# Intsights/PySubstringSearch

Hardware: AMD Instinct MI355X
Metric: queries/sec (batched) + index-build GB/s on 512MB chunk, 1/2/4/8 GPU (higher is better)
Workload: dtype u64

## Files before the change

pysubstringsearch_amd/csrc/common.cpp:

```cpp
#include "common.h"
#include "knobs.h"

#include <atomic>
#include <cstring>
#include <cstdio>
#include <cstdlib>
#include <algorithm>
#include <cerrno>
#include <unistd.h>

#include <mutex>
#include <vector>

namespace pss {

static thread_local std::string g_err;

void set_error(const char *fmt, ...)
{
    char buf[1024];
    va_list ap;
    va_start(ap, fmt);
    vsnprintf(buf, sizeof buf, fmt, ap);
    va_end(ap);
// ... 294 lines not shown
    if (e != hipSuccess || count <= 0) {
        (void)hipGetLastError();
        set_error("no usable HIP device (%s); libpss has no CPU fallback",
                  e != hipSuccess ? hipGetErrorString(e) : "device count is 0");
        return PSS_EDEVICE;
    }
    if (device < 0 || device >= count || device >= kMaxDevices) {
        set_error("device %d out of range (have %d)", device, count);
        return PSS_EINVAL;
    }
    PSS_HIP(hipSetDevice(device));
    std::lock_guard<std::mutex> lk(g_ctx_mu);
    DeviceCtx &c = table[device];
    if (c.device < 0) PSS_TRY(init_ctx(c, device));
    *out = &c;
    return PSS_OK;
}

int get_helper_ctx(DeviceCtx *parent, DeviceCtx **out)
{
    if (!parent->helper) {
        DeviceCtx *h = new DeviceCtx();
        const int rc = init_ctx(*h, parent->device);
        if (rc != PSS_OK) {
            delete h;
            return rc;
        }
        parent->helper = h;
    }
    *out = parent->helper;
    return PSS_OK;
}

int get_ctx(int device, DeviceCtx **out) { return get_ctx_of(g_ctx, device, out); }
int get_build_ctx(int device, DeviceCtx **out) { return get_ctx_of(g_bctx, device, out); }

int DeviceCtx::ensure_resident()
{
    if (resident.arena) return PSS_OK;
    PSS_HIP(hipStreamCreateWithFlags(&resident.stream, hipStreamNonBlocking));
    PSS_HIP(hipHostMalloc(&resident.arena, kPinnedBytes, hipHostMallocCoherent | hipHostMallocMapped));
    PSS_HIP(hipHostGetDevicePointer(&resident.arena_dev, resident.arena, 0));
    memset(resident.arena, 0, kPinnedBytes);
    return PSS_OK;
}

void DeviceCtx::Resident::post(const uint8_t *q, uint32_t plen)
{
    ResidentMailbox *mb = reinterpret_cast<ResidentMailbox *>(static_cast<uint8_t *>(arena) + kResidentMailboxOff);
    if (plen != kResidentStop) {
        if (plen <= sizeof mb->post.bytes) {
            memcpy(mb->post.bytes, q, plen);
        } else {
            memcpy(mb->query, q, plen);
            memset(mb->query + plen, 0, 32);
        }
    }
    mb->post.plen = plen;
    ++seq;
    __atomic_store_n(&mb->post.seq_b, seq, __ATOMIC_RELEASE);
    __atomic_store_n(&mb->post.seq_a, seq, __ATOMIC_RELEASE);
}

void DeviceCtx::stop_resident()
{
    if (!resident.running) return;
    resident.post(nullptr, kResidentStop);
    (void)hipStreamSynchronize(resident.stream);
    resident.running = false;
}

const KnobDef kKnobs[] = {
    {"PSS_KEY_CHARS", "0 (chosen)", "1|2|3|5|8|12|16", "builder: force the symbols packed into the initial sort key"},
    {"PSS_KEY_DROP", "-1 (chosen)", "0|1|3|7", "builder: force the low bits of the last key symbol that are left out"},
    {"PSS_NO_SAMPLE", "unset", "1", "builder: size the initial key from symbol counts even for large texts (no sizing sample)"},
    {"PSS_NO_TIES_PASS", "unset", "1", "builder: plain 8-byte-key LSD passes and key comparison in the rerank (no tie flags)"},
    {"PSS_MODE", "chosen", "dense|sparse|text", "builder: how ties are resolved -- doubling over an inverse suffix array, sparse (hash), text rounds"},
    {"PSS_TEXT_ROUNDS", "5", "0|1|2|3", "builder: text rounds at most before the rank rounds"},
    {"PSS_MSD", "-1 (screened)", "0|1|1", "initial sort: never / whenever the key fits the hybrid MSD radix sort (msd_sort.hip)"},
    {"PSS_MSD_LSD", "1", "0|1", "MSD sort: 0 = digits in MSD order with a second histogram pass (rounds 2-5); else LSD order, second pass by look-back"},
    {"PSS_MSD_KEY_CAP", "48", "", "MSD sort: largest key width tried (bits; the element format bounds it further)"},
    {"PSS_MSD_PARTIAL_SYMBOL", "unset", "1", "MSD sort: fill the element with the high bits of one more symbol than fits whole (fewer ties; measured slower on lines)"},
    {"PSS_MSD_NO_FUSE", "unset", "1", "MSD sort: ties flagged in the suffix array instead of emitted from the local sort"},
    {"PSS_MSD_SLOW_LOCAL", "unset", "1", "MSD sort: the general (ballot LSD) local-sort kernel for every tile"},
    {"PSS_MSD_SCATTER", "unset", "1", "MSD sort in MSD order: the 8192-element partition kernels of round 2"},
    {"PSS_SS", "-1 (n >= 2^24, MSD declined)", "0|1", "initial sort: never / whenever the text has the size for it the sample sort over 16-byte elements"},
    {"PSS_SS_SEG", "1", "0", "sample sort: 0 = every tile merge-sorted as one array instead of bucket by bucket"},
    {"PSS_SS_WINDOW_PLAN", "unset", "1", "sample sort: tiles by the window rule of the MSD sort instead of the greedy plan"},
    {"PSS_SS_DEBUG", "unset", "", "sample sort: print where a bucket beyond a tile came from (diagnostic)"},
    {"PSS_NO_PLAN_CACHE", "unset", "1", "builder: forget between chunks which initial sort and alphabet the previous chunk took"},
    {"PSS_NO_PLAN_FRONT", "unset", "1", "builder: remember the sort but not the alphabet (separate alphabet and recode passes)"},
    {"PSS_RLE", "-1 (runs average >= 8 bytes)", "0|1|1", "builder: never / always the run-length path (rle_build.hip)"},
    {"PSS_RLE_SORT", "unset", "1", "run-length path: expansion by the stable radix sort instead of the matrix walk"},
    {"PSS_PERIOD", "-1 (when the text repeats one word)", "0", "builder: 0 = never the closed form for a text that repeats one word"},
    {"PSS_ANCHOR", "-1 (texts of >= 2^20 bytes)", "0|1|1", "builder: never / whenever ties outlive the text rounds the anchor round (anchor_impl.h)"},
    {"PSS_ANCHOR_OMEGA", "0 (as wide as the common prefix allows)", "9|12|17|33", "anchor round: force the window of the minimizers"},
    {"PSS_ANCHOR_MIN_OMEGA", "11", "3|7|9", "anchor round: narrowest window it accepts by itself"},
    {"PSS_ANCHOR_SIDE", "-1 (>= 2^24 bytes, sampled ties show copies)", "0|1", "anchor round: never / always sort the anchors beside the text round (second stream)"},
    {"PSS_ANCHOR_SIDE_PCT", "8", "", "anchor round: share of sampled tied pairs that must be copies for the side line"},
    {"PSS_ANCHOR_CAP_DIV", "5", "3|4", "anchor round: declines above n / this many anchors"},
    {"PSS_NO_PROBE", "unset", "1", "builder: always a text round before the anchor round (no sampling of the ties)"},
    {"PSS_PROBE_SKIP_PCT", "50", "0|20|90", "builder: no text rounds when more than this share of the sampled tied pairs are repeats"},
    {"PSS_NO_MID_TIER", "unset", "1", "rounds: groups above 512 members all take the chained radix sorts"},
    {"PSS_NO_MID_MERGE", "unset", "1", "rounds: groups of 513 .. 4096 members with a crowded bin take the chained sorts (no LDS merge sort)"},
    {"PSS_BIG_MERGE", "-1 (by the average size of the large groups)", "0|1|2", "rounds: groups above 4096 members through the segmented merge sort (2: in text rounds only)"},
    {"PSS_NO_BIG_MERGE", "unset", "", "rounds: overrides PSS_BIG_MERGE"},
    {"PSS_COUNT_SORT", "unset", "1", "rank rounds: groups ranked by counting instead of the merge sort"},
    {"PSS_PERIODIC", "1", "0", "rank rounds: 0 = no periodic keys for the large groups"},
    {"PSS_TIMING", "unset", "", "builder / Writer: per-round and per-stage trace on stderr"},
    {"PSS_DEVICES", "all visible", "0|0,0|0,0,0|all", "devices of Reader(path) / Writer(path) without a device argument: all | comma-separated ordinals"},
    {"PSS_DEVICE", "unset", "", "default device of a process (launchers' LOCAL_RANK etc. are honoured the same way)"},
    {"PSS_IO_THREADS", "8 .. 16 by core count", "2|5", "file path: threads of the I/O pool"},
    {"PSS_INGEST_BLOCK", "32 MiB", "16|40|300", "Writer: size of the direct reads of add_entries_from_file_lines"},
    {"PSS_INGEST_MIN_ROOM", "1 MiB", "1|20", "Writer: room a chunk must have left for one direct read"},
    {"PSS_WRITER_MMAP", "tmpfs: 1, else 0", "0|1", "Writer: records through a shared mapping (1) or pwrite (0)"},
    {"PSS_WRITER_MMAP_MIN", "1 MiB", "16", "Writer: smallest record that goes through the mapping"},
    {"PSS_WRITER_HOST_BUDGET", "8 GiB", "", "multi-device Writer: host text of the chunks in flight (one chunk always goes through)"},
    {"PSS_STRIPES", "8", "", "striped container format 2: stripe files of a Writer"},
    {"PSS_EXPERIMENT_NO_FILE", "unset", "", "measurement only: the record thread copies without writing the file"},
    {"PSS_RESULT_ORDER", "text", "sa", "Reader: 'sa' = the reference's order inside a chunk (suffix-array order of every entry's first hit)"},
    {"PSS_READER_HBM_BUDGET", "whatever hipMalloc grants minus 2 GiB", "", "Reader: suffix arrays beyond this many bytes of HBM stay in pinned host memory"},
    {"PSS_READER_AUTO_RESIDENCY", "1", "", "Reader: 0 = the residency manager never moves a suffix array by itself"},
    {"PSS_NO_KEY_SAMPLES", "unset", "", "Reader: no key-sample table"},
    {"PSS_SAMPLE_SHIFT", "11", "", "Reader: one key sample per 2^shift suffixes"},
    {"PSS_LINE_BLOCK_SHIFT", "8", "6|7|9|10", "Reader: the line index behind entry ids keeps one newline rank per 2^shift bytes of text (6 .. 10)"},
    {"PSS_NO_SMALL_PATH", "unset", "1", "search: no fused single-query kernels"},
    {"PSS_NO_BLOCK_PATH", "unset", "1", "search: small batches one wave per pair instead of one workgroup"},
    {"PSS_NO_SEARCH_STAGE", "unset", "1", "search: no pinned staging of queries and results"},
    {"PSS_WAVE_SEARCH", "unset", "1", "search: interval kernel one wave per pair at every batch size"},
    {"PSS_NO_GROUP_SEARCH", "unset", "1", "search: never 16 lanes per pair"},
    {"PSS_NO_MID_PIPELINE", "unset", "1", "search: always the general multi-kernel pipeline"},
    {"PSS_PINNED_POOL_BYTES", "40 GiB", "", "search: pinned host memory the result pool keeps between batches"},
    {"PSS_NO_PINNED_RESULTS", "unset", "1", "search: large results into pageable memory"},
    {"PSS_LANE_SEARCH_MIN", "8192", "1|100000", "search: pairs from which one lane per pair searches"},
    {"PSS_SEARCH_EVENTS", "unset", "", "single-query path: HIP events around the fused kernel (fills ms_device; ~4 us per query)"},
    {"PSS_RESIDENT_IDLE_US", "1000", "", "low-latency mode: the resident kernel leaves after this long without a query"},
    {"PSS_RESIDENT_LIFE_US", "50000", "", "low-latency mode: ... and after this long in any case"},
    {"PSS_TRACE_RESIDENT", "unset", "", "libpss_trace.so only: print the resident kernel's phase stamps"},
    {"PSS_RCCL_LIB", "librccl.so of the process", "", "gather inside the C ABI: the RCCL library to load"},
    {"PSS_RCCL_TIMEOUT_MS", "60000", "", "gather inside the C ABI: bound of every wait for the peers"},
};
const int kNumKnobs = (int)(sizeof(kKnobs) / sizeof(kKnobs[0]));

const char *knob(const char *name)
{
    for (int i = 0; i < kNumKnobs; ++i)
        if (strcmp(kKnobs[i].name, name) == 0) return getenv(name);
    static std::atomic<bool> said{false};
    if (!said.exchange(true)) fprintf(stderr, "[pss] %s is not in the switch registry (knobs.h): treated as unset\n", name);
    return nullptr;
}

uint64_t workspace_bytes(int device)
{
    if (device < 0 || device >= kMaxDevices) return 0;
    std::lock_guard<std::mutex> lk(g_ctx_mu);
    uint64_t total = 0;
    for (DeviceCtx *table : {g_ctx, g_bctx}) {
        DeviceCtx &c = table[device];
        if (c.device < 0) continue;
        for (auto &s : c.slot) total += s.cap;
        if (c.helper)
            for (auto &s : c.helper->slot) total += s.cap;
    }
    return total;
}
// ... 27 lines not shown
```

pysubstringsearch_amd/csrc/msd_sort.hip:

```cpp
#include "msd_sort.h"

#include <algorithm>
#include <vector>

#include "prims.h"
#include "scan.h"
#include "text_keys.h"

namespace pss {

constexpr int MSD_D = 10;
constexpr u32 MSD_BINS = 1u << MSD_D;
constexpr int MSD_BLOCK = 512;
constexpr int MSD_WAVES = MSD_BLOCK / kWave;
constexpr int MSD_IPT = 16;
constexpr u32 MSD_TILE = MSD_BLOCK * MSD_IPT;
constexpr u32 MSD_WIN = 6144;
#ifndef PSS_LS_WINDOW
#define PSS_LS_WINDOW 8
#endif
constexpr u32 MSD_TILE_CAP = 8184 - PSS_LS_WINDOW;
constexpr u32 MSD_MAX_BUCKET = 4088;
constexpr int MSD_TAG_BITS = MSD_D + 1;
constexpr u32 MSD_TAG_SPAN = 1u << MSD_TAG_BITS;
// ... 522 lines not shown
                        e = ((e >> 24) << a.idx_bits) | (u64)(base + ((u32)e & (MSD_TILE2 - 1u)));
                    } else {
                        d = (u32)(e >> shift2) & (MSD_BINS - 1u);
                        e = (e & low_mask2) | ((u64)(hist[d] >> 16) << shift2);
                    }
                    a.out[s_delta[d] + p] = e;
                }
            }
        }
    }
}

constexpr u32 LB_A = 1u << 30, LB_P = 2u << 30, LB_STATE = 3u << 30, LB_VALUE = LB_A - 1u;
constexpr int LB_WINDOW = 4;

struct LbAsk {
    u32 v[LB_WINDOW];
};
__device__ __forceinline__ void lb_ask(const u32 *status, u32 p, LbAsk &q)
{
#pragma unroll
    for (u32 w = 0; w < (u32)LB_WINDOW; ++w) {
        const u32 r = p > w ? p - 1 - w : 0u;
        q.v[w] = __hip_atomic_load(&status[(size_t)r * MSD_BINS + threadIdx.x], __ATOMIC_RELAXED, __HIP_MEMORY_SCOPE_AGENT);
    }
}
__device__ __forceinline__ void lb_begin(u32 *status, u32 t, u32 c, LbAsk &q)
{
    if (t == 0) return;
    __hip_atomic_store(&status[(size_t)t * MSD_BINS + threadIdx.x], LB_A | c, __ATOMIC_RELAXED, __HIP_MEMORY_SCOPE_AGENT);
    lb_ask(status, t, q);
}
__device__ __forceinline__ u32 lb_finish(u32 *status, u32 t, u32 c, u32 first, LbAsk &q)
{
    u32 off = first;
    if (t != 0) {
        u32 sum = 0, p = t;
        for (;;) {
            const u32 p0 = p;
            bool stop = false, done = false;
#pragma unroll
            for (u32 w = 0; w < (u32)LB_WINDOW; ++w) {
                if (!stop && w < p0) {
                    const u32 st = q.v[w] & LB_STATE;
                    if (st == 0) {
                        stop = true;
                    } else {
                        sum += q.v[w] & LB_VALUE;
                        --p;
                        if (st == LB_P) done = stop = true;
                    }
                }
            }
            if (done || p == 0) break;
            lb_ask(status, p, q);
        }
        off = sum;
    }
    __hip_atomic_store(&status[(size_t)t * MSD_BINS + threadIdx.x], LB_P | (off + c), __ATOMIC_RELAXED, __HIP_MEMORY_SCOPE_AGENT);
    return off;
}


__global__ __launch_bounds__(MSD_BINS) void msd_tiles2_kernel(const u32 *J1, MsdTile2 *tiles, u32 *counters)
{
    __shared__ u32 scr[MSD_BINS / kWave + 1];
    const u32 d = threadIdx.x;
    const u32 s = J1[d], e = J1[d + 1];
    const u32 nr = (e - s + MSD_TILE2 - 1) / MSD_TILE2;
    u32 total = 0, D = 0;
    const u32 first = block_excl_sum<MSD_BINS / kWave>(nr, scr, &total);
    const u32 dn = block_excl_sum<MSD_BINS / kWave>(nr ? 1u : 0u, scr, &D);
    if (d == 0) counters[0] = total + (MSD_BINS - D);
    if (nr == 0) {
        const u32 dd = D + (d - dn);
        tiles[total + (d - dn)] = MsdTile2{s, 0u, dd | 0x80000000u};
    }
    for (u32 k = 0; k < nr; ++k) {
        const u32 ts = s + k * MSD_TILE2;
        tiles[first + k] = MsdTile2{ts, min(MSD_TILE2, e - ts), dn | (k + 1 == nr ? 0x80000000u : 0u)};
    }
}

__global__ __launch_bounds__(1024) void msd_scatter_lb_kernel(MsdArgs a)
{
    constexpr int BLOCK = 1024;
    constexpr int IPT = MSD_TILE2 / BLOCK;
    __shared__ __attribute__((aligned(16))) u64 exch[MSD_TILE];
    __shared__ u32 hist[MSD_BINS], s_delta[MSD_BINS];
    __shared__ u16 s_start[MSD_BINS];
    __shared__ u32 scr[BLOCK / kWave + 1];
    __shared__ u32 s_ticket;
    const u32 tid = threadIdx.x;
    const u32 nt = a.counters[0];
    const int shift2 = a.idx_bits + a.key_bits - 2 * MSD_D;
    const u64 low_mask2 = (1ull << shift2) - 1ull;
    hist[tid] = 0;
    __syncthreads();
    for (;;) {
        if (tid == 0) s_ticket = atomicAdd(&a.counters[8], 1u);
        __syncthreads();
        const u32 t = s_ticket;
        if (t >= nt) break;
        const MsdTile2 td = a.tiles2[t];
        const u32 base = td.start, valid = td.count;
        u64 elem[IPT];
        u32 lp[IPT];
#pragma unroll
        for (int k = 0; k < IPT; ++k) {
            const u32 p = k * BLOCK + tid;
            elem[k] = p < valid ? a.in[base + p] : 0ull;
        }
#pragma unroll
        for (int k = 0; k < IPT; ++k) {
            const u32 p = k * BLOCK + tid;
            const u32 d = (u32)(elem[k] >> shift2) & (MSD_BINS - 1u);
            lp[k] = p < valid ? (atomicAdd(&hist[d], 1u) | (d << 22)) : 0xffffffffu;
        }
        __syncthreads();
        const u32 c = hist[tid];
        LbAsk ask;
        lb_begin(a.status, t, c, ask);
        const u32 ex = block_excl_sum<BLOCK / kWave>(c, scr, nullptr);
        s_start[tid] = (u16)ex;
        hist[tid] = 0;
        __syncthreads();
        const u64 tag = (u64)(td.d_last & (MSD_RAW_TAG_SPAN - 1u)) << shift2;
#pragma unroll
        for (int k = 0; k < IPT; ++k)
            if (lp[k] != 0xffffffffu) lp[k] = (lp[k] & 0xffffu) + (u32)s_start[lp[k] >> 22];
#pragma unroll
        for (int h = 0; h < MSD_PIECES2; ++h) {
            if (h && h * MSD_TILE >= valid) break;
            if (h) __syncthreads();
#pragma unroll
            for (int k = 0; k < IPT; ++k) {
                const u32 q = lp[k] - h * MSD_TILE;
                if (q < MSD_TILE) exch[q] = elem[k];
            }
            if (h == 0) {
                if (t == 0 && tid == 0) a.J[0] = 0;
                const u32 off = lb_finish(a.status, t, c, a.Jb[tid], ask);
                if (td.d_last >> 31) a.J[(size_t)tid * MSD_BINS + (td.d_last & (MSD_BINS - 1u)) + 1u] = off + c;
                s_delta[tid] = off - ex;
            }
            __syncthreads();
#pragma unroll
            for (int k = 0; k < (int)(MSD_TILE / BLOCK); ++k) {
                const u32 q = k * BLOCK + tid, p = h * MSD_TILE + q;
                if (p < valid) {
                    const u64 e = exch[q];
                    const u32 d = (u32)(e >> shift2) & (MSD_BINS - 1u);
                    a.out[s_delta[d] + p] = (e & low_mask2) | tag;
                }
            }
        }
    }
}


struct InNonEmpty {
    const u32 *J;
    __device__ u64 operator()(u64 j) const { return J[j + 1] > J[j] ? 1u : 0u; }
};

__global__ __launch_bounds__(256) void msd_compact_kernel(const u32 *J, u32 nb, const u64 *rank, u32 *cstart, u32 *counters, u32 *cj)
{
    u32 mx = 0;
    for (u32 j = blockIdx.x * blockDim.x + threadIdx.x; j < nb; j += gridDim.x * blockDim.x) {
        const u32 s = J[j], e = J[j + 1];
        if (e > s) {
            cstart[rank[j]] = s;
            if (cj) cj[rank[j]] = j;
            mx = max(mx, e - s);
        }
    }
    mx = wave_incl_max(mx);
    if (lane_id() == kWave - 1 && mx) atomicMax(&counters[1], mx);
}

struct TilePlan {
    u32 win, cap;
    const u32 *cj;
};
__device__ __forceinline__ bool msd_tile_head(const u32 *cstart, u32 ne, u32 n, u32 k, TilePlan tp)
{
    if (tp.cj) {
        if (k == 0 || (tp.cj[k] >> MSD_RAW_TAG_BITS) != (tp.cj[k - 1] >> MSD_RAW_TAG_BITS)) return true;
    } else if ((k & (MSD_TAG_SPAN - 1u)) == 0) {
        return true;
    }
    const u32 w = cstart[k] / tp.win;
    if (cstart[k - 1] / tp.win != w) return true;
    if (k + 1 < ne && cstart[k + 1] / tp.win == w) return false;
    u32 lo = 0, hi = k;
    const u32 ws = w * tp.win;
    while (lo < hi) {
        const u32 mid = (lo + hi) >> 1;
        if (cstart[mid] < ws) lo = mid + 1; else hi = mid;
    }
    const u32 end = k + 1 < ne ? cstart[k + 1] : n;
    return end - cstart[lo] > tp.cap;
}

struct InTileHead {
    const u32 *cstart;
    u32 ne, n;
    TilePlan tp;
    __device__ u64 operator()(u64 k) const { return msd_tile_head(cstart, ne, n, (u32)k, tp) ? 1u : 0u; }
};

struct InTileHeadDev {
    const u32 *cstart;
    const u64 *nep;
    u32 n;
    TilePlan tp;
    __device__ u64 operator()(u64 k) const
    {
        const u32 ne = (u32)*nep;
        return (k < ne && msd_tile_head(cstart, ne, n, (u32)k, tp)) ? 1u : 0u;
    }
};
__global__ __launch_bounds__(256) void msd_tiles_dev_kernel(const u32 *cstart, const u64 *nep, u32 n, const u64 *rank, const u64 *total,
                                                              u32 *tile_first, TilePlan tp)
{
    const u32 ne = (u32)*nep;
    if (blockIdx.x == 0 && threadIdx.x == 0) tile_first[*total] = ne;
    for (u32 k = blockIdx.x * blockDim.x + threadIdx.x; k < ne; k += gridDim.x * blockDim.x) {
        if (msd_tile_head(cstart, ne, n, k, tp)) tile_first[rank[k]] = k;
    }
}

// ... 148 lines not shown
                for (int w = 0; w < MSD_WAVES; ++w) {
                    c[w] = wave_hist[w][tid];
                    total += c[w];
                }
            }
            const u32 incl = wave_incl_sum(total);
            if (lane == kWave - 1) scr[wave] = incl;
            __syncthreads();
            if (tid < 256) {
                u32 run = incl - total;
                for (u32 w = 0; w < wave; ++w) run += scr[w];
#pragma unroll
                for (int w = 0; w < MSD_WAVES; ++w) {
                    wave_hist[w][tid] = run;
                    run += c[w];
                }
            }
        }
        __syncthreads();
#pragma unroll
        for (int r = 0; r < MSD_IPT; ++r) {
            const bool pad = wave * (kWave * MSD_IPT) + r * kWave + lane >= count;
            const u32 d = pad ? dmask : ((u32)(key[r] >> shift) & dmask);
            exch[wave_hist[wave][d] + rank[r]] = key[r];
        }
        __syncthreads();
        for (u32 i = tid; i < MSD_WAVES * 256; i += MSD_BLOCK) (&wave_hist[0][0])[i] = 0;
#pragma unroll
        for (int r = 0; r < MSD_IPT; ++r) key[r] = exch[wave * (kWave * MSD_IPT) + r * kWave + lane];
        __syncthreads();
    }
    if (sort_bits <= 0) {
#pragma unroll
        for (int r = 0; r < MSD_IPT; ++r) exch[wave * (kWave * MSD_IPT) + r * kWave + lane] = key[r];
        __syncthreads();
    }
    if (tid == 0) scr[0] = 0;
    __syncthreads();
    msd_emit_tile(exch, count, e0, idx_bits, sa_out, em, &scr[0]);
    __syncthreads();
    if (em && tid == 0) em->blk_cnt[t] = scr[0];
}


#ifndef PSS_LS_BIN_BITS
#define PSS_LS_BIN_BITS 12
#endif
constexpr int LS_BIN_BITS = PSS_LS_BIN_BITS;
constexpr u32 LS_BINS = 1u << LS_BIN_BITS;
constexpr u32 LS_WORDS = LS_BINS / 2;
constexpr u32 LS_KMAX = 64;
#ifndef PSS_LS_GROUP
#define PSS_LS_GROUP 1
#endif
constexpr int LS_GROUP = PSS_LS_GROUP;
constexpr int LS_WINDOW = PSS_LS_WINDOW;

__global__ __launch_bounds__(256) void msd_tile_desc_kernel(const u32 *cstart, const u32 *tile_first, u32 nt, u32 ne, u32 n,
                                                              MsdTile *tiles, const u32 *cj, const u64 *ntp, const u64 *nep)
{
    const u32 t = blockIdx.x * blockDim.x + threadIdx.x;
    if (ntp) {
        nt = (u32)*ntp;
        ne = (u32)*nep;
    }
    if (t >= nt) return;
    const u32 k0 = tile_first[t], k1 = tile_first[t + 1];
    const u32 e0 = cstart[k0], e1 = k1 < ne ? cstart[k1] : n;
    if (cj) {
        const u32 t0 = cj[k0] & (MSD_RAW_TAG_SPAN - 1u), t1 = cj[k1 - 1] & (MSD_RAW_TAG_SPAN - 1u);
        tiles[t] = MsdTile{e0, e1 - e0, t0, t1 - t0 + 1u};
    } else {
        tiles[t] = MsdTile{e0, e1 - e0, k0 & (MSD_TAG_SPAN - 1u), k1 - k0};
    }
}

__device__ __forceinline__ void keep_load(u64 &v) { asm volatile("" : "+v"(v)); }

__device__ __forceinline__ void lds_barrier()
{
    asm volatile("s_waitcnt lgkmcnt(0)\n\ts_barrier" ::: "memory");
}

__global__ __launch_bounds__(MSD_BLOCK, 4) void msd_local_fast_kernel(const u64 *in, const MsdTile *tiles, u32 nt, int rem_bits,
                                                                     int idx_bits, u32 *sa_out, u32 *fail_list, u32 *fail_count,
                                                                     int fused, MsdEmit em_val, const u64 *nt_dev,
                                                                     const u32 *counters_dev, const u32 *bad_dev)
{
    if (nt_dev) {
        if (counters_dev[1] > MSD_MAX_BUCKET || (bad_dev && *bad_dev)) return;
        nt = (u32)*nt_dev;
    }
    const MsdEmit *em = fused ? &em_val : nullptr;
    __shared__ __attribute__((aligned(16))) u64 lds_all[MSD_TILE + LS_WORDS];
    u64 *const exch = lds_all;
    u32 *const hist = reinterpret_cast<u32 *>(lds_all + MSD_TILE);
    u32 *const hist2 = hist + LS_WORDS;
    u32 *const scr = reinterpret_cast<u32 *>(&exch[MSD_TILE - 8]);
    u32 &s_fail = scr[MSD_WAVES + 2];
    const u32 tid = threadIdx.x;
    const u32 stride = gridDim.x;
    u32 t = blockIdx.x;
    if (t >= nt) return;
    MsdTile cur = tiles[t];
    MsdTile nxt = t + stride < nt ? tiles[t + stride] : MsdTile{0, 0, 0, 0};
    u64 pe[MSD_IPT];
    auto prefetch = [&](const MsdTile &d) {
#pragma unroll
        for (int r = 0; r < MSD_IPT; ++r) {
            const u32 p = r * MSD_BLOCK + tid;
            pe[r] = p < d.count ? in[d.e0 + p] : 0ull;
        }
    };
    prefetch(cur);
    for (u32 i = tid; i < LS_WORDS; i += MSD_BLOCK) hist[i] = 0;
    if (tid == 0) {
        s_fail = 0;
        scr[MSD_WAVES + 3] = 0;
    }
    lds_barrier();
    u32 prev_t = 0;
    bool prev_ok = false;
    for (;;) {
        const u32 count = cur.count, e0 = cur.e0;
        const u32 rows = (count + MSD_BLOCK - 1) / MSD_BLOCK;
        int seg_bits = 0;
        while ((1u << seg_bits) < cur.nb) ++seg_bits;
        const u64 tag_base = (u64)cur.tag0 << (rem_bits + idx_bits);
        const int sort_bits = rem_bits + seg_bits;
        const int bin_shift = idx_bits + (sort_bits > LS_BIN_BITS ? sort_bits - LS_BIN_BITS : 0);
        u64 e[MSD_IPT];
#pragma unroll
        for (int r = 0; r < MSD_IPT; ++r) {
            e[r] = ~0ull;
            if ((u32)r < rows) {
                const u32 p = r * MSD_BLOCK + tid;
                if (p < count) {
                    e[r] = pe[r] - tag_base;
                    const u32 bin = (u32)(e[r] >> bin_shift);
                    atomicAdd(&hist[bin >> 1], 1u << (16u * (bin & 1u)));
                }
            }
        }
        const bool more = t + stride < nt;
        if (more) prefetch(nxt);
        lds_barrier();
        if (tid == 0) {
            if (em && prev_ok) em->blk_cnt[prev_t] = scr[MSD_WAVES + 3];
            s_fail = 0;
            scr[MSD_WAVES + 3] = 0;
        }
        {
            constexpr int LS_WPT = LS_WORDS / MSD_BLOCK;
            static_assert(LS_WPT * MSD_BLOCK == (int)LS_WORDS && LS_WPT >= 1, "bins split evenly over the threads");
            u32 c[2 * LS_WPT];
            u32 sum = 0;
#pragma unroll
            for (int j = 0; j < LS_WPT; ++j) {
                const u32 wv = hist[LS_WPT * tid + j];
                c[2 * j] = wv & 0xffffu;
                c[2 * j + 1] = wv >> 16;
                sum += c[2 * j] + c[2 * j + 1];
            }
            const u32 incl = wave_incl_sum(sum);
            if (lane_id() == kWave - 1) scr[wave_id()] = incl;
            lds_barrier();
            u32 ex = incl - sum;
            for (int w = 0; w < wave_id(); ++w) ex += scr[w];
#pragma unroll
            for (int j = 0; j < LS_WPT; ++j) {
                const u32 lo = ex, hi = ex + c[2 * j];
                hist[LS_WPT * tid + j] = hist2[LS_WPT * tid + j] = lo | (hi << 16);
                ex = hi + c[2 * j + 1];
            }
        }
        lds_barrier();
#pragma unroll
        for (int r = 0; r < MSD_IPT; ++r) {
            if ((u32)r < rows) {
                const u32 p = r * MSD_BLOCK + tid;
                if (p < count) {
                    const u32 bin = (u32)(e[r] >> bin_shift), sh = 16u * (bin & 1u);
                    exch[(atomicAdd(&hist2[bin >> 1], 1u << sh) >> sh) & 0xffffu] = e[r];
                }
            }
        }
        if (tid < (u32)LS_WINDOW) exch[count + tid] = ~0ull;
        lds_barrier();
        const u16 *const starts16 = reinterpret_cast<const u16 *>(hist);
        u32 rk[MSD_IPT];
#pragma unroll
        for (int g = 0; g < MSD_IPT; g += LS_GROUP) {
            if ((u32)g < rows) {
                u64 x[LS_GROUP];
                u32 s0[LS_GROUP], sm[LS_GROUP];
#pragma unroll
                for (int j = 0; j < LS_GROUP; ++j) x[j] = exch[(g + j) * MSD_BLOCK + tid];
#pragma unroll
                for (int j = 0; j < LS_GROUP; ++j) {
                    const u32 bin = (u32)(x[j] >> bin_shift) & (LS_BINS - 1u);
                    s0[j] = starts16[bin];
                }
                u64 y[LS_GROUP][LS_WINDOW];
#pragma unroll
                for (int j = 0; j < LS_GROUP; ++j) {
#pragma unroll
                    for (int k = 0; k < LS_WINDOW; ++k) y[j][k] = exch[s0[j] + k];
                }
#pragma unroll
                for (int j = 0; j < LS_GROUP; ++j) {
                    u32 c = 0;
#pragma unroll
                    for (int k = 0; k < LS_WINDOW; ++k) {
                        keep_load(y[j][k]);
                        c += y[j][k] < x[j] ? 1u : 0u;
                    }
                    sm[j] = c;
                }
#pragma unroll
                for (int j = 0; j < LS_GROUP; ++j) {
                    const u32 p = (g + j) * MSD_BLOCK + tid;
                    if (p < count && ((y[j][LS_WINDOW - 1] ^ x[j]) >> bin_shift) == 0) {
                        const u32 bin = (u32)(x[j] >> bin_shift) & (LS_BINS - 1u);
                        const u32 s1 = bin + 1u < LS_BINS ? (u32)starts16[min(bin + 1u, LS_BINS - 1u)] : count;
                        const u32 len = s1 - s0[j];
                        if (len > LS_KMAX) {
                            s_fail = 1;
                        } else {
                            for (u32 q = s0[j] + LS_WINDOW; q < s0[j] + len; ++q) sm[j] += exch[q] < x[j] ? 1u : 0u;
                        }
                    }
                    e[g + j] = x[j];
                    rk[g + j] = s0[j] + sm[j];
                }
            } else {
#pragma unroll
                for (int j = 0; j < LS_GROUP; ++j) rk[g + j] = 0;
            }
        }
        lds_barrier();
        const bool failed = s_fail != 0;
        if (failed) {
            if (tid == 0) fail_list[atomicAdd(fail_count, 1u)] = t;
        } else {
#pragma unroll
            for (int r = 0; r < MSD_IPT; ++r) {
                if ((u32)r < rows) {
                    const u32 p = r * MSD_BLOCK + tid;
                    if (p < count) exch[rk[r]] = e[r];
                }
            }
        }
        for (u32 i = tid; i < LS_WORDS; i += MSD_BLOCK) hist[i] = 0;
        lds_barrier();
        if (!failed) {
            const u32 imask = (u32)((1ull << idx_bits) - 1ull);
            u32 *const s_count = &scr[MSD_WAVES + 3];
#pragma unroll
            for (int g = 0; g < MSD_IPT; g += LS_GROUP) {
                if ((u32)g < rows) {
                    u64 cur[LS_GROUP], prv[LS_GROUP], nxt[LS_GROUP];
#pragma unroll
                    for (int j = 0; j < LS_GROUP; ++j) {
                        const u32 p = (g + j) * MSD_BLOCK + tid;
                        cur[j] = exch[p];
                        prv[j] = exch[p ? p - 1 : 0];
                        nxt[j] = exch[p + 1];
                    }
#pragma unroll
                    for (int j = 0; j < LS_GROUP; ++j) {
                        keep_load(cur[j]);
                        keep_load(prv[j]);
                        keep_load(nxt[j]);
                    }
#pragma unroll
                    for (int j = 0; j < LS_GROUP; ++j) {
                        const u32 p = (g + j) * MSD_BLOCK + tid;
                        if (p < count) {
                            const u64 kx = cur[j] >> idx_bits;
                            const bool tie = p > 0 && (prv[j] >> idx_bits) == kx;
                            const u32 sfx = (u32)cur[j] & imask;
                            sa_out[e0 + p] = sfx | ((tie && em == nullptr) ? 0x80000000u : 0u);
                            if (em != nullptr) {
                                const bool tie_next = p + 1 < count && (nxt[j] >> idx_bits) == kx;
                                if (tie || tie_next) {
                                    const u32 slot = e0 + atomicAdd(s_count, 1u);
                                    em->st_pos[slot] = e0 + p;
                                    em->st_idx[slot] = sfx | (tie ? 0x80000000u : 0u);
                                }
                            }
                        }
                    }
                }
            }
        }
        prev_t = t;
        prev_ok = !failed;
        if (!more) break;
        t += stride;
        cur = nxt;
        nxt = t + stride < nt ? tiles[t + stride] : MsdTile{0, 0, 0, 0};
    }
    if (em) {
        lds_barrier();
        if (tid == 0 && prev_ok) em->blk_cnt[prev_t] = scr[MSD_WAVES + 3];
    }
}

#include "ss_sort_impl.h"


static size_t msd_max_tiles(uint32_t n)
{
    return (size_t)n / (SS_WIN / 2) + ((size_t)MSD_BINS * MSD_BINS) / MSD_RAW_TAG_SPAN + 8;
}

static size_t msd_max_tiles2(uint32_t n) { return (size_t)n / MSD_TILE2 + MSD_BINS + 8; }

static bool msd_use_lsd(uint32_t n)
{
    const char *e = knob("PSS_MSD_LSD");
    return !(e && atoi(e) == 0) && n < (1u << 30);
}

size_t msd_workspace_bytes(uint32_t n)
{
    const size_t max_ranges2 = (size_t)n / MSD_G2_RANGE + MSD_BINS + 8;
    const size_t nbk = (size_t)MSD_BINS * MSD_BINS;
    return max_ranges2 * MSD_BINS * 4
           + (MSD_BINS + 8) * 4
           + (nbk + 8) * 4
           + max_ranges2 * sizeof(MsdRange) + (MSD_BINS + 8) * 4 + 64
           + (nbk + 8) * 8
           + (nbk + 8) * 4
           + (msd_max_tiles(n) + 32) * 8
           + (msd_max_tiles(n) + 32) * 16
           + (msd_max_tiles(n) + 32) * sizeof(MsdTile)
           + (SC_MAX_BLOCKS + 8) * 8 + 8192
           + (size_t)MSD_BINS * MSD_G1_RANGES * 4 + (MSD_BINS + 8) * 4
           + msd_max_tiles2(n) * (sizeof(MsdTile2) + (size_t)MSD_BINS * 4)
           + (nbk + 8) * 4 + 4096;
}

int msd_max_key_bits(uint32_t n)
{
    int ib = 1;
    while ((1ull << ib) < (u64)n) ++ib;
    const int after2 = 64 + MSD_D - (msd_use_lsd(n) ? MSD_RAW_TAG_BITS : MSD_TAG_BITS) - ib + MSD_D;
    return std::min(after2, 64 + MSD_D - ib);
}

int msd_suffix_sort(DeviceCtx *ctx, const TextKeys *text, uint32_t n, int key_bits, uint64_t *A[2], uint32_t *sa_out,
                    void *work, uint32_t *h_small, bool profile, MsdStats *stats, bool *accepted, MsdActive *active,
                    const MsdFront *front)
{
    *accepted = false;
    hipStream_t s = ctx->stream;
    int ib = 1;
    while ((1ull << ib) < (u64)n) ++ib;
    if (key_bits < 2 * MSD_D + 1 || key_bits > msd_max_key_bits(n) || n < 2) {
        set_error("msd_suffix_sort: key of %d bits does not fit (n = %u)", key_bits, n);
        return PSS_EINVAL;
    }
    const size_t max_ranges2 = (size_t)n / MSD_G2_RANGE + MSD_BINS + 8;
    const size_t nbk = (size_t)MSD_BINS * MSD_BINS;
    u8 *w = static_cast<u8 *>(work);
    size_t o = 0;
    auto carve = [&](size_t bytes) { u8 *p = w + o; o = round_up(o + bytes, 256); return p; };
    u32 *T = reinterpret_cast<u32 *>(carve(max_ranges2 * MSD_BINS * 4));
    u32 *J1 = reinterpret_cast<u32 *>(carve((MSD_BINS + 8) * 4));
    u32 *J = reinterpret_cast<u32 *>(carve((nbk + 8) * 4));
    MsdRange *ranges2 = reinterpret_cast<MsdRange *>(carve(max_ranges2 * sizeof(MsdRange)));
    u32 *seg_first = reinterpret_cast<u32 *>(carve((MSD_BINS + 8) * 4));
    u32 *counters = reinterpret_cast<u32 *>(carve(64));
    u64 *ranks = reinterpret_cast<u64 *>(carve((nbk + 8) * 8));
    u32 *cstart = reinterpret_cast<u32 *>(carve((nbk + 8) * 4));
    const size_t max_tiles = msd_max_tiles(n);
    MsdTile *tiles_all = reinterpret_cast<MsdTile *>(carve((max_tiles + 16) * sizeof(MsdTile)));
    u32 *tile_first = reinterpret_cast<u32 *>(carve((max_tiles + 16) * 8));
    u32 *blk_cnt = reinterpret_cast<u32 *>(carve((max_tiles + 8) * 4));
    u64 *dst_off = reinterpret_cast<u64 *>(carve((max_tiles + 8) * 8));
    u64 *partial = reinterpret_cast<u64 *>(carve((SC_MAX_BLOCKS + 8) * 8));
    u64 *d_total = partial + SC_MAX_BLOCKS;
    const bool lsd = msd_use_lsd(n);
    const size_t max_tiles2 = msd_max_tiles2(n);
    u32 *T2 = nullptr, *Jb = nullptr, *status = nullptr, *cj = nullptr;
    MsdTile2 *tiles2 = nullptr;
    if (lsd) {
        T2 = reinterpret_cast<u32 *>(carve((size_t)MSD_BINS * MSD_G1_RANGES * 4));
        Jb = reinterpret_cast<u32 *>(carve((MSD_BINS + 8) * 4));
        tiles2 = reinterpret_cast<MsdTile2 *>(carve(max_tiles2 * sizeof(MsdTile2)));
        status = reinterpret_cast<u32 *>(carve(max_tiles2 * MSD_BINS * 4));
        cj = reinterpret_cast<u32 *>(carve((nbk + 8) * 4));
    }

    MsdArgs a;
    memset(&a, 0, sizeof a);
    a.codes = text->codes;
    a.code_bits = text->code_bits;
    a.key_chars = text->key_chars;
    a.plus_one = text->plus_one;
    a.key_drop = text->drop;
    a.n = n;
    a.key_bits = key_bits;
    a.idx_bits = ib;
    const u32 num_tiles = (u32)(((u64)n + MSD_TILE - 1) / MSD_TILE);
    a.tiles_per_range1 = (num_tiles + MSD_G1_RANGES - 1) / MSD_G1_RANGES;
    a.num_ranges1 = (num_tiles + a.tiles_per_range1 - 1) / a.tiles_per_range1;
    a.T = T;
    a.J1 = J1;
    a.J = J;
    a.ranges2 = ranges2;
    a.seg_first = seg_first;
    a.counters = counters;
    a.lsd = lsd ? 1 : 0;
    a.T2 = T2;
    a.Jb = Jb;
    a.tiles2 = tiles2;
    a.status = status;

    hipEvent_t ev[8] = {};
    int nev = 0;
    struct EvGuard {
        hipEvent_t *e;
        int *n;
        ~EvGuard()
        {
            for (int i = 0; i < *n; ++i) (void)hipEventDestroy(e[i]);
        }
    } guard{ev, &nev};
    auto mark = [&]() -> int {
        if (profile && nev < 8) {
            PSS_HIP(hipEventCreate(&ev[nev]));
            PSS_HIP(hipEventRecord(ev[nev], s));
            ++nev;
        }
        return PSS_OK;
    };

    PSS_HIP(hipMemsetAsync(counters, 0, 64, s));
    a.out = A[0];
    if (front) {
        a.raw = front->raw;
        a.lut = front->lut;
        a.codes_out = const_cast<u8 *>(text->codes);
        a.bad = front->bad;
        hipLaunchKernelGGL(msd_hist_raw_kernel, dim3(a.num_ranges1), dim3(MSD_BLOCK), 0, s, a);
    } else {
        hipLaunchKernelGGL(msd_hist_kernel<true>, dim3(a.num_ranges1), dim3(MSD_BLOCK), 0, s, a);
    }
    static_assert(MSD_G1_RANGES <= 1024, "msd_offsets1_kernel takes four ranges per thread");
    hipLaunchKernelGGL(msd_offsets1_kernel, dim3(MSD_BINS), dim3(256), 0, s, T, a.num_ranges1, seg_first);
    hipLaunchKernelGGL(msd_offsets1b_kernel, dim3(1), dim3(MSD_BINS), 0, s, (const u32 *)seg_first, J1, n);
    if (lsd) {
        hipLaunchKernelGGL(msd_offsets1_kernel, dim3(MSD_BINS), dim3(256), 0, s, T2, a.num_ranges1, seg_first);
        hipLaunchKernelGGL(msd_offsets1b_kernel, dim3(1), dim3(MSD_BINS), 0, s, (const u32 *)seg_first, Jb, n);
        PSS_HIP(hipMemsetAsync(status, 0, max_tiles2 * MSD_BINS * 4, s));
    }
    PSS_TRY(mark());
    const bool wide = lsd || !(knob("PSS_MSD_SCATTER") && atoi(knob("PSS_MSD_SCATTER")) == 1);
    if (lsd) hipLaunchKernelGGL((msd_scatter2_kernel<true, 1024, true>), dim3(a.num_ranges1), dim3(1024), 0, s, a);
    else if (wide) hipLaunchKernelGGL((msd_scatter2_kernel<true, 1024>), dim3(a.num_ranges1), dim3(1024), 0, s, a);
    else hipLaunchKernelGGL(msd_scatter_kernel<true>, dim3(a.num_ranges1), dim3(MSD_BLOCK), 0, s, a);
    PSS_TRY(mark());
    a.in = A[0];
    a.out = A[1];
    if (lsd) {
        hipLaunchKernelGGL(msd_tiles2_kernel, dim3(1), dim3(MSD_BINS), 0, s, (const u32 *)J1, tiles2, counters);
        PSS_TRY(mark());
        const u32 grid2 = std::min<u32>((u32)max_tiles2, (u32)ctx->num_cus);
        hipLaunchKernelGGL(msd_scatter_lb_kernel, dim3(grid2), dim3(1024), 0, s, a);
        PSS_TRY(mark());
    } else {
        hipLaunchKernelGGL(msd_ranges_kernel, dim3(1), dim3(MSD_BINS), 0, s, J1, ranges2, seg_first, counters);
        a.dense = ranks;
        hipLaunchKernelGGL(msd_hist_kernel<false>, dim3((u32)max_ranges2), dim3(MSD_BLOCK), 0, s, a);
        hipLaunchKernelGGL(msd_offsets_kernel, dim3(MSD_BINS), dim3(MSD_BINS), 0, s, T, (const u32 *)seg_first, (const u32 *)J1, J,
                           0u, n, MSD_BINS);
    }
    PSS_TRY(device_excl_scan(ctx, InNonEmpty{J}, nbk, partial, d_total, ranks));
    hipLaunchKernelGGL(msd_compact_kernel, dim3(1024), dim3(256), 0, s, J, (u32)nbk, ranks, cstart, counters, cj);
    const int rem_bits = key_bits - 2 * MSD_D;
    MsdEmit em{};
    const int fused = active != nullptr;
    if (fused) em = MsdEmit{active->st_pos, active->st_idx, blk_cnt};
    const bool one_trip = lsd && !knob("PSS_MSD_SLOW_LOCAL");
    u64 *d_total2 = d_total + 1;
    u32 *const fail_list_dev = tile_first + max_tiles + 16;
    if (one_trip) {
        const TilePlan tpd{MSD_WIN, MSD_TILE_CAP, cj};
        PSS_TRY(device_excl_scan(ctx, InTileHeadDev{cstart, d_total, n, tpd}, nbk, partial, d_total2, ranks));
        hipLaunchKernelGGL(msd_tiles_dev_kernel, dim3(1024), dim3(256), 0, s, cstart, (const u64 *)d_total, n, ranks, (const u64 *)d_total2,
                           tile_first, tpd);
        hipLaunchKernelGGL(msd_tile_desc_kernel, dim3((u32)((max_tiles + 255) / 256)), dim3(256), 0, s, cstart, tile_first, 0u, 0u, n,
                           tiles_all, (const u32 *)cj, (const u64 *)d_total2, (const u64 *)d_total);
        PSS_TRY(mark());
        hipLaunchKernelGGL(msd_local_fast_kernel, dim3(2u * (u32)ctx->num_cus), dim3(MSD_BLOCK), 0, s, A[1], (const MsdTile *)tiles_all, 0u,
                           rem_bits, ib, sa_out, fail_list_dev, counters + 4, fused, em, (const u64 *)d_total2, (const u32 *)counters,
                           front ? (const u32 *)front->bad : (const u32 *)nullptr);
        PSS_TRY(mark());
        PSS_HIP(hipMemcpyAsync(h_small + 8, d_total2, 8, hipMemcpyDeviceToHost, s));
        PSS_HIP(hipMemcpyAsync(h_small + 10, counters + 4, 4, hipMemcpyDeviceToHost, s));
    }
    PSS_HIP(hipMemcpyAsync(h_small, d_total, 8, hipMemcpyDeviceToHost, s));
    PSS_HIP(hipMemcpyAsync(h_small + 2, counters, 16, hipMemcpyDeviceToHost, s));
    if (front) PSS_HIP(hipMemcpyAsync(h_small + 6, front->bad, 4, hipMemcpyDeviceToHost, s));
    PSS_HIP(hipStreamSynchronize(s));
    const u32 ne = h_small[0];
    const u32 maxb = h_small[3];
    if (stats) {
        stats->buckets = ne;
        stats->max_bucket = maxb;
        stats->bad_symbol = front ? h_small[6] : 0u;
    }
    if (front && h_small[6]) return PSS_OK;
    if (maxb > MSD_MAX_BUCKET) return PSS_OK;
    if (!lsd) {
        PSS_TRY(mark());
        if (wide) hipLaunchKernelGGL((msd_scatter2_kernel<false, 1024>), dim3((u32)max_ranges2), dim3(1024), 0, s, a);
        else hipLaunchKernelGGL(msd_scatter_kernel<false>, dim3((u32)max_ranges2), dim3(MSD_BLOCK), 0, s, a);
        PSS_TRY(mark());
    }
    const auto local_sort = msd_local_sort_kernel;
    const auto local_fast = msd_local_fast_kernel;
    u32 nt = 0;
    u32 *fail_list = fail_list_dev;
    if (one_trip) {
        nt = h_small[8];
        if ((size_t)nt > max_tiles) {
            set_error("msd_suffix_sort: %u tiles planned, tables hold %zu (internal error)", nt, max_tiles);
            return PSS_EDEVICE;
        }
        const u32 nfail = h_small[10];
        if (stats) stats->slow_tiles = nfail;
        if (nfail)
            hipLaunchKernelGGL(local_sort, dim3(nfail), dim3(MSD_BLOCK), 0, s, A[1], (const MsdTile *)tiles_all, rem_bits,
                               ib, sa_out, (const u32 *)fail_list, fused, em);
    } else {
    const TilePlan tp{MSD_WIN, MSD_TILE_CAP, cj};
    PSS_TRY(device_excl_scan(ctx, InTileHead{cstart, ne, n, tp}, ne, partial, d_total, ranks));
    hipLaunchKernelGGL(msd_tiles_kernel, dim3(1024), dim3(256), 0, s, cstart, ne, n, ranks, (const u64 *)d_total, tile_first, tp);
    PSS_HIP(hipMemcpyAsync(h_small, d_total, 8, hipMemcpyDeviceToHost, s));
    PSS_HIP(hipStreamSynchronize(s));
    nt = h_small[0];
    if ((size_t)nt > max_tiles) {
        set_error("msd_suffix_sort: %u tiles planned, tables hold %zu (internal error)", nt, max_tiles);
        return PSS_EDEVICE;
    }
    PSS_TRY(mark());
    fail_list = tile_first + nt + 8;
    hipLaunchKernelGGL(msd_tile_desc_kernel, dim3((nt + 255) / 256), dim3(256), 0, s, cstart, tile_first, nt, ne, n, tiles_all,
                       (const u32 *)cj, (const u64 *)nullptr, (const u64 *)nullptr);
    if (knob("PSS_MSD_SLOW_LOCAL")) {
        hipLaunchKernelGGL(local_sort, dim3(nt), dim3(MSD_BLOCK), 0, s, A[1], (const MsdTile *)tiles_all, rem_bits, ib,
                           sa_out, (const u32 *)nullptr, fused, em);
    } else {
        MsdTile *tiles = tiles_all;
        const u32 grid = std::min<u32>(nt, 2u * (u32)ctx->num_cus);
        hipLaunchKernelGGL(local_fast, dim3(grid), dim3(MSD_BLOCK), 0, s, A[1], (const MsdTile *)tiles, nt, rem_bits, ib,
                           sa_out, fail_list, counters + 4, fused, em, (const u64 *)nullptr, (const u32 *)nullptr, (const u32 *)nullptr);
        PSS_TRY(mark());
        PSS_HIP(hipMemcpyAsync(h_small, counters + 4, 4, hipMemcpyDeviceToHost, s));
        PSS_HIP(hipStreamSynchronize(s));
        const u32 nfail = h_small[0];
        if (stats) stats->slow_tiles = nfail;
        if (nfail)
            hipLaunchKernelGGL(local_sort, dim3(nfail), dim3(MSD_BLOCK), 0, s, A[1], (const MsdTile *)tiles_all, rem_bits,
                               ib, sa_out, (const u32 *)fail_list, fused, em);
    }
    if (knob("PSS_MSD_SLOW_LOCAL")) PSS_TRY(mark());
    }
    if (fused) {
        PSS_TRY(device_excl_scan(ctx, InBlkCnt{blk_cnt}, nt, partial, d_total, dst_off));
        hipLaunchKernelGGL(msd_gather_kernel, dim3((nt + 3) / 4), dim3(256), 0, s, (const MsdTile *)tiles_all, blk_cnt, dst_off, nt,
                           active->st_pos, active->st_idx, active->pos, active->idx, active->grp);
        PSS_HIP(hipMemcpyAsync(h_small, d_total, 8, hipMemcpyDeviceToHost, s));
        PSS_HIP(hipStreamSynchronize(s));
        active->count = h_small[0];
    }
    PSS_HIP(hipGetLastError());
    if (stats) {
        stats->tiles = nt;
        stats->lookback = lsd ? 1u : 0u;
    }
    if (profile && nev >= 6) {
        PSS_HIP(hipStreamSynchronize(s));
        float ms = 0.f;
        PSS_HIP(hipEventElapsedTime(&ms, ev[0], ev[1]));
        if (stats) stats->ms_g1 = ms;
        PSS_HIP(hipEventElapsedTime(&ms, ev[2], ev[3]));
        if (stats) stats->ms_g2 = ms;
        PSS_HIP(hipEventElapsedTime(&ms, ev[4], ev[5]));
        if (stats) stats->ms_local = ms;
    }
    *accepted = true;
    return PSS_OK;
}


struct SsGeometry {
    u32 B1, B2, os, S;
    int ib, kc, key_bits;
    u64 plo, phi;
};
static bool ss_geometry(uint32_t n, uint32_t radix, SsGeometry *g)
{
    if (n < (1u << 16) || n > (1u << 30) || radix < 2 || radix > 257) return false;
// ... 269 lines not shown
```

Baseline: 65.93.

## Use 32-bit key forms in fast local sort and one-piece look-back staging

Templates the fast local-sort kernel so that when the index bits fit in 32 bits, bin extraction, tag subtraction and key equality use 32-bit halves instead of 64-bit shifts. The tie emission in the fused path now reads a neighbour through a wave ballot rather than loading the next element per lane. Separately, the look-back scatter kernel can stage its whole tile in LDS at once instead of in pieces, which removes barriers but raises LDS use per block. Both are on by default through a new knob, which can select the previous paths.

Result: slower. 64.41 (-2.3%).

```diff
diff --git a/pysubstringsearch_amd/csrc/common.cpp b/pysubstringsearch_amd/csrc/common.cpp
--- a/pysubstringsearch_amd/csrc/common.cpp
+++ b/pysubstringsearch_amd/csrc/common.cpp
@@ -400,6 +400,7 @@
     {"PSS_MSD_KEY_CAP", "48", "", "MSD sort: largest key width tried (bits; the element format bounds it further)"},
     {"PSS_MSD_PARTIAL_SYMBOL", "unset", "1", "MSD sort: fill the element with the high bits of one more symbol than fits whole (fewer ties; measured slower on lines)"},
     {"PSS_MSD_NO_FUSE", "unset", "1", "MSD sort: ties flagged in the suffix array instead of emitted from the local sort"},
+    {"PSS_MSD_R7", "3", "0|1|2", "MSD sort: bit 0 = 32-bit forms in the fast local sort, bit 1 = the look-back pass stages its tile in one piece; 0 = both as in round 6"},
     {"PSS_MSD_SLOW_LOCAL", "unset", "1", "MSD sort: the general (ballot LSD) local-sort kernel for every tile"},
     {"PSS_MSD_SCATTER", "unset", "1", "MSD sort in MSD order: the 8192-element partition kernels of round 2"},
     {"PSS_SS", "-1 (n >= 2^24, MSD declined)", "0|1", "initial sort: never / whenever the text has the size for it the sample sort over 16-byte elements"},
diff --git a/pysubstringsearch_amd/csrc/msd_sort.hip b/pysubstringsearch_amd/csrc/msd_sort.hip
--- a/pysubstringsearch_amd/csrc/msd_sort.hip
+++ b/pysubstringsearch_amd/csrc/msd_sort.hip
@@ -628,11 +628,14 @@
     }
 }
 
+template <bool ONE_PIECE>
 __global__ __launch_bounds__(1024) void msd_scatter_lb_kernel(MsdArgs a)
 {
     constexpr int BLOCK = 1024;
     constexpr int IPT = MSD_TILE2 / BLOCK;
-    __shared__ __attribute__((aligned(16))) u64 exch[MSD_TILE];
+    constexpr u32 PIECE = ONE_PIECE ? MSD_TILE2 : MSD_TILE;
+    constexpr int PIECES = (int)(MSD_TILE2 / PIECE);
+    __shared__ __attribute__((aligned(16))) u64 exch[PIECE];
     __shared__ u32 hist[MSD_BINS], s_delta[MSD_BINS];
     __shared__ u16 s_start[MSD_BINS];
     __shared__ u32 scr[BLOCK / kWave + 1];
@@ -676,13 +679,13 @@
         for (int k = 0; k < IPT; ++k)
             if (lp[k] != 0xffffffffu) lp[k] = (lp[k] & 0xffffu) + (u32)s_start[lp[k] >> 22];
 #pragma unroll
-        for (int h = 0; h < MSD_PIECES2; ++h) {
-            if (h && h * MSD_TILE >= valid) break;
+        for (int h = 0; h < PIECES; ++h) {
+            if (h && h * PIECE >= valid) break;
             if (h) __syncthreads();
 #pragma unroll
             for (int k = 0; k < IPT; ++k) {
-                const u32 q = lp[k] - h * MSD_TILE;
-                if (q < MSD_TILE) exch[q] = elem[k];
+                const u32 q = lp[k] - h * PIECE;
+                if (q < PIECE) exch[q] = elem[k];
             }
             if (h == 0) {
                 if (t == 0 && tid == 0) a.J[0] = 0;
@@ -692,8 +695,8 @@
             }
             __syncthreads();
 #pragma unroll
-            for (int k = 0; k < (int)(MSD_TILE / BLOCK); ++k) {
-                const u32 q = k * BLOCK + tid, p = h * MSD_TILE + q;
+            for (int k = 0; k < (int)(PIECE / BLOCK); ++k) {
+                const u32 q = k * BLOCK + tid, p = h * PIECE + q;
                 if (p < valid) {
                     const u64 e = exch[q];
                     const u32 d = (u32)(e >> shift2) & (MSD_BINS - 1u);
@@ -1008,6 +1011,26 @@
     asm volatile("s_waitcnt lgkmcnt(0)\n\ts_barrier" ::: "memory");
 }
 
+template <bool HI>
+__device__ __forceinline__ u32 ls_bin(u64 e, int bin_shift)
+{
+    if constexpr (HI) return (u32)(e >> 32) >> (bin_shift - 32);
+    else return (u32)(e >> bin_shift);
+}
+template <bool HI>
+__device__ __forceinline__ bool ls_same_bin(u64 a, u64 b, int bin_shift)
+{
+    if constexpr (HI) return (((u32)(a >> 32) ^ (u32)(b >> 32)) >> (bin_shift - 32)) == 0;
+    else return ((a ^ b) >> bin_shift) == 0;
+}
+template <bool W32>
+__device__ __forceinline__ bool ls_same_key(u64 a, u64 b, int idx_bits)
+{
+    if constexpr (W32) return ((u32)(a >> 32) == (u32)(b >> 32)) & ((((u32)a ^ (u32)b) >> idx_bits) == 0);
+    else return (a >> idx_bits) == (b >> idx_bits);
+}
+
+template <bool W32, bool HI>
 __global__ __launch_bounds__(MSD_BLOCK, 4) void msd_local_fast_kernel(const u64 *in, const MsdTile *tiles, u32 nt, int rem_bits,
                                                                      int idx_bits, u32 *sa_out, u32 *fail_list, u32 *fail_count,
                                                                      int fused, MsdEmit em_val, const u64 *nt_dev,
@@ -1053,6 +1076,7 @@
         int seg_bits = 0;
         while ((1u << seg_bits) < cur.nb) ++seg_bits;
         const u64 tag_base = (u64)cur.tag0 << (rem_bits + idx_bits);
+        const u32 tag_hi = (u32)(tag_base >> 32);
         const int sort_bits = rem_bits + seg_bits;
         const int bin_shift = idx_bits + (sort_bits > LS_BIN_BITS ? sort_bits - LS_BIN_BITS : 0);
         u64 e[MSD_IPT];
@@ -1062,8 +1086,9 @@
             if ((u32)r < rows) {
                 const u32 p = r * MSD_BLOCK + tid;
                 if (p < count) {
-                    e[r] = pe[r] - tag_base;
-                    const u32 bin = (u32)(e[r] >> bin_shift);
+                    if constexpr (HI) e[r] = ((u64)((u32)(pe[r] >> 32) - tag_hi) << 32) | (u32)pe[r];
+                    else e[r] = pe[r] - tag_base;
+                    const u32 bin = ls_bin<HI>(e[r], bin_shift);
                     atomicAdd(&hist[bin >> 1], 1u << (16u * (bin & 1u)));
                 }
             }
@@ -1106,7 +1131,7 @@
             if ((u32)r < rows) {
                 const u32 p = r * MSD_BLOCK + tid;
                 if (p < count) {
-                    const u32 bin = (u32)(e[r] >> bin_shift), sh = 16u * (bin & 1u);
+                    const u32 bin = ls_bin<HI>(e[r], bin_shift), sh = 16u * (bin & 1u);
                     exch[(atomicAdd(&hist2[bin >> 1], 1u << sh) >> sh) & 0xffffu] = e[r];
                 }
             }
@@ -1124,7 +1149,7 @@
                 for (int j = 0; j < LS_GROUP; ++j) x[j] = exch[(g + j) * MSD_BLOCK + tid];
 #pragma unroll
                 for (int j = 0; j < LS_GROUP; ++j) {
-                    const u32 bin = (u32)(x[j] >> bin_shift) & (LS_BINS - 1u);
+                    const u32 bin = ls_bin<HI>(x[j], bin_shift) & (LS_BINS - 1u);
                     s0[j] = starts16[bin];
                 }
                 u64 y[LS_GROUP][LS_WINDOW];
@@ -1146,8 +1171,8 @@
 #pragma unroll
                 for (int j = 0; j < LS_GROUP; ++j) {
                     const u32 p = (g + j) * MSD_BLOCK + tid;
-                    if (p < count && ((y[j][LS_WINDOW - 1] ^ x[j]) >> bin_shift) == 0) {
-                        const u32 bin = (u32)(x[j] >> bin_shift) & (LS_BINS - 1u);
+                    if (p < count && ls_same_bin<HI>(y[j][LS_WINDOW - 1], x[j], bin_shift)) {
+                        const u32 bin = ls_bin<HI>(x[j], bin_shift) & (LS_BINS - 1u);
                         const u32 s1 = bin + 1u < LS_BINS ? (u32)starts16[min(bin + 1u, LS_BINS - 1u)] : count;
                         const u32 len = s1 - s0[j];
                         if (len > LS_KMAX) {
@@ -1182,37 +1207,70 @@
         if (!failed) {
             const u32 imask = (u32)((1ull << idx_bits) - 1ull);
             u32 *const s_count = &scr[MSD_WAVES + 3];
-#pragma unroll
-            for (int g = 0; g < MSD_IPT; g += LS_GROUP) {
-                if ((u32)g < rows) {
-                    u64 cur[LS_GROUP], prv[LS_GROUP], nxt[LS_GROUP];
-#pragma unroll
-                    for (int j = 0; j < LS_GROUP; ++j) {
-                        const u32 p = (g + j) * MSD_BLOCK + tid;
-                        cur[j] = exch[p];
-                        prv[j] = exch[p ? p - 1 : 0];
-                        nxt[j] = exch[p + 1];
-                    }
-#pragma unroll
-                    for (int j = 0; j < LS_GROUP; ++j) {
-                        keep_load(cur[j]);
-                        keep_load(prv[j]);
-                        keep_load(nxt[j]);
-                    }
-#pragma unroll
-                    for (int j = 0; j < LS_GROUP; ++j) {
-                        const u32 p = (g + j) * MSD_BLOCK + tid;
-                        if (p < count) {
-                            const u64 kx = cur[j] >> idx_bits;
-                            const bool tie = p > 0 && (prv[j] >> idx_bits) == kx;
-                            const u32 sfx = (u32)cur[j] & imask;
-                            sa_out[e0 + p] = sfx | ((tie && em == nullptr) ? 0x80000000u : 0u);
-                            if (em != nullptr) {
-                                const bool tie_next = p + 1 < count && (nxt[j] >> idx_bits) == kx;
+            if constexpr (W32) {
+                const u32 lane = lane_id();
+                const bool last_lane = lane == (u32)kWave - 1u;
+#pragma unroll
+                for (int g = 0; g < MSD_IPT; ++g) {
+                    if ((u32)g < rows) {
+                        const u32 p = g * MSD_BLOCK + tid;
+                        u64 cur = exch[p], prv = exch[p ? p - 1 : 0], nxt = 0;
+                        if (em != nullptr && last_lane) nxt = exch[p + 1];
+                        keep_load(cur);
+                        keep_load(prv);
+                        const bool in = p < count;
+                        const bool tie = in & (p > 0) & ls_same_key<true>(prv, cur, idx_bits);
+                        const u32 sfx = (u32)cur & imask;
+                        if (em == nullptr) {
+                            if (in) sa_out[e0 + p] = sfx | (tie ? 0x80000000u : 0u);
+                        } else {
+                            const u64 ties = __builtin_amdgcn_ballot_w64(tie);
+                            bool tie_next = ((u32)((ties >> 1) >> lane) & 1u) != 0;
+                            if (last_lane) tie_next = (p + 1 < count) & ls_same_key<true>(nxt, cur, idx_bits);
+                            if (in) {
+                                sa_out[e0 + p] = sfx;
                                 if (tie || tie_next) {
                                     const u32 slot = e0 + atomicAdd(s_count, 1u);
                                     em->st_pos[slot] = e0 + p;
                                     em->st_idx[slot] = sfx | (tie ? 0x80000000u : 0u);
+                                }
+                            }
+                        }
+                    }
+                }
+            } else {
+#pragma unroll
+                for (int g = 0; g < MSD_IPT; g += LS_GROUP) {
+                    if ((u32)g < rows) {
+                        u64 cur[LS_GROUP], prv[LS_GROUP], nxt[LS_GROUP];
+#pragma unroll
+                        for (int j = 0; j < LS_GROUP; ++j) {
+                            const u32 p = (g + j) * MSD_BLOCK + tid;
+                            cur[j] = exch[p];
+                            prv[j] = exch[p ? p - 1 : 0];
+                            nxt[j] = exch[p + 1];
+                        }
+#pragma unroll
+                        for (int j = 0; j < LS_GROUP; ++j) {
+                            keep_load(cur[j]);
+                            keep_load(prv[j]);
+                            keep_load(nxt[j]);
+                        }
+#pragma unroll
+                        for (int j = 0; j < LS_GROUP; ++j) {
+                            const u32 p = (g + j) * MSD_BLOCK + tid;
+                            if (p < count) {
+                                const u64 kx = cur[j] >> idx_bits;
+                                const bool tie = p > 0 && (prv[j] >> idx_bits) == kx;
+                                const u32 sfx = (u32)cur[j] & imask;
+                                sa_out[e0 + p] = sfx | ((tie && em == nullptr) ? 0x80000000u : 0u);
+                                if (em != nullptr) {
+                                    const bool tie_next = p + 1 < count && (nxt[j] >> idx_bits) == kx;
+                                    if (tie || tie_next) {
+                                        const u32 slot = e0 + atomicAdd(s_count, 1u);
+                                        em->st_pos[slot] = e0 + p;
+                                        em->st_idx[slot] = sfx | (tie ? 0x80000000u : 0u);
+                                    }
                                 }
                             }
                         }
@@ -1364,6 +1422,12 @@
         return PSS_OK;
     };
 
+    const char *r7e = knob("PSS_MSD_R7");
+    const int r7 = r7e ? atoi(r7e) : 3;
+    const int rem_bits = key_bits - 2 * MSD_D;
+    const bool l_w32 = (r7 & 1) && ib < 32;
+    const bool l_hi = l_w32 && ib + std::max(0, rem_bits - LS_BIN_BITS) >= 32;
+    const auto local_fast = l_hi ? msd_local_fast_kernel<true, true> : l_w32 ? msd_local_fast_kernel<true, false> : msd_local_fast_kernel<false, false>;
     PSS_HIP(hipMemsetAsync(counters, 0, 64, s));
     a.out = A[0];
     if (front) {
@@ -1395,7 +1459,8 @@
         hipLaunchKernelGGL(msd_tiles2_kernel, dim3(1), dim3(MSD_BINS), 0, s, (const u32 *)J1, tiles2, counters);
         PSS_TRY(mark());
         const u32 grid2 = std::min<u32>((u32)max_tiles2, (u32)ctx->num_cus);
-        hipLaunchKernelGGL(msd_scatter_lb_kernel, dim3(grid2), dim3(1024), 0, s, a);
+        if (r7 & 2) hipLaunchKernelGGL(msd_scatter_lb_kernel<true>, dim3(grid2), dim3(1024), 0, s, a);
+        else hipLaunchKernelGGL(msd_scatter_lb_kernel<false>, dim3(grid2), dim3(1024), 0, s, a);
         PSS_TRY(mark());
     } else {
         hipLaunchKernelGGL(msd_ranges_kernel, dim3(1), dim3(MSD_BINS), 0, s, J1, ranges2, seg_first, counters);
@@ -1406,7 +1471,6 @@
     }
     PSS_TRY(device_excl_scan(ctx, InNonEmpty{J}, nbk, partial, d_total, ranks));
     hipLaunchKernelGGL(msd_compact_kernel, dim3(1024), dim3(256), 0, s, J, (u32)nbk, ranks, cstart, counters, cj);
-    const int rem_bits = key_bits - 2 * MSD_D;
     MsdEmit em{};
     const int fused = active != nullptr;
     if (fused) em = MsdEmit{active->st_pos, active->st_idx, blk_cnt};
@@ -1421,7 +1485,7 @@
         hipLaunchKernelGGL(msd_tile_desc_kernel, dim3((u32)((max_tiles + 255) / 256)), dim3(256), 0, s, cstart, tile_first, 0u, 0u, n,
                            tiles_all, (const u32 *)cj, (const u64 *)d_total2, (const u64 *)d_total);
         PSS_TRY(mark());
-        hipLaunchKernelGGL(msd_local_fast_kernel, dim3(2u * (u32)ctx->num_cus), dim3(MSD_BLOCK), 0, s, A[1], (const MsdTile *)tiles_all, 0u,
+        hipLaunchKernelGGL(local_fast, dim3(2u * (u32)ctx->num_cus), dim3(MSD_BLOCK), 0, s, A[1], (const MsdTile *)tiles_all, 0u,
                            rem_bits, ib, sa_out, fail_list_dev, counters + 4, fused, em, (const u64 *)d_total2, (const u32 *)counters,
                            front ? (const u32 *)front->bad : (const u32 *)nullptr);
         PSS_TRY(mark());
@@ -1448,7 +1512,6 @@
         PSS_TRY(mark());
     }
     const auto local_sort = msd_local_sort_kernel;
-    const auto local_fast = msd_local_fast_kernel;
     u32 nt = 0;
     u32 *fail_list = fail_list_dev;
     if (one_trip) {
```
